# linwe2012/CourseComputationalPhotography

Hardware: AMD Instinct MI355X
Metric: Gauss-Seidel pixel-updates/s on WxH 5-point Poisson grid (higher is better)
Workload: dtype f64

## Files before the change

### coursecomputationalphotography_amd/csrc/ccp_grid.hip

```cpp
#include "ccp_grid_kernels.hpp"
#include "ccp_grid_fused.hpp"
#include "ccp_grid_fused_wide.hpp"
#include "ccp_grid_lex.hpp"
#include "ccp_cg.hpp"
#include "ccp_grid_cg.hpp"
#include "ccp_grid_mg_view.hpp"
#include "ccp_grid_blend.hpp"
#include "ccp_grid_weighted.hpp"
#include "ccp_comm.hpp"

#include <algorithm>
#include <functional>
#include <cstring>
#include <chrono>
#include <vector>

using namespace ccp;

constexpr int kEdgeRing = 64;

struct ccp_grid {
    ccp_grid_desc desc{};
    Geom geom{};
    int ghost_top = 0, ghost_bottom = 0;
    bool shrink_top = false, shrink_bottom = false;
    int device = 0;
    hipStream_t stream = nullptr;
    hipStream_t stream2 = nullptr;
    hipEvent_t ev_main = nullptr, ev_side = nullptr;
    unsigned long long *edge_counter = nullptr;
    unsigned long long *edge_flag = nullptr;
    unsigned long long edge_epoch = 0;
    unsigned *edge_timeout = nullptr;
    unsigned long long edge_timeout_ticks = 200000000ull;
    int wait_mode = 0;
    bool edge_signal = true;
    ccp_comm *comm = nullptr;
    std::vector<int> part;
    int up_rank = -1, down_rank = -1;
    int send_up = 0, send_down = 0;
    hipStream_t stream_comm = nullptr;
    hipEvent_t ev_comm = nullptr, ev_ready = nullptr;
    bool overlap = true;
    long exchanges = 0;
    DevBuf<double> x, b;
    DevBuf<double> cg_r, cg_p, cg_p2, cg_ap;
    DevBuf<CgState> cg_state;
    DevBuf<double> x_alt;
    bool allow_swap = false;
    bool masked = false;
    DevBuf<unsigned char> maskp, tile_live;
    DevBuf<int> tile_rows;
    DevBuf<unsigned char> mask_edge;
    bool mask_edge_known = false;
    int mask_border = -1;
    int live_T = -1, live_R = -1, live_lo = -1, live_hi = -1;
    long unknowns = 0;
    bool fuse = true;
    int multi = 0;
    DevBuf<unsigned> multi_words;
    bool xcd_swizzle = false;
    const char *trace_file = nullptr;
    DevBuf<unsigned long long> trace;
    bool short_edges = true;
    int side_rows_override = 0;
    int fuse_tmax = kFusedMaxT;
    int rows_per_chunk = 128;
    float tune_ms[kFusedMaxT + 1] = {0};
    int tune_rows[kFusedMaxT + 1] = {0};
    bool tuned = false;
    bool all_border = false;
    bool force_border = false;
    bool red_store_all = false;
    bool wide = true;
    DevBuf<double> partial;
    long partial_region = 0;
    DevBuf<double> small;
    DevBuf<unsigned> io_bad;
    DevBuf<double> sweep_sums;
    DevBuf<SolveState> state;
    DevBuf<int> redo_mask;
    DevBuf<double> lex_x, lex_b, lex_snap, lex_partial, lex_eps;
    DevBuf<unsigned> lex_progress, lex_ticket;
    DevBuf<double> lex_edges;
    int lex_mode = 3;
    int lex_tmax = 8;
    unsigned *lex_order_pin = nullptr;
    unsigned *lex_order_dev = nullptr;
    size_t lex_order_pin_cap = 0;
    size_t lex_order_count = 0;
    int lex_order_groups = 0, lex_order_strips = 0, lex_order_depth = 0;
    LexGeom lexg{};
    DevBuf<double> stage;
    long stage_rows = 0;
    int half_sweeps_since_refresh = 0;
    hipEvent_t ev0 = nullptr, ev1 = nullptr;
    hipEvent_t ev_r0 = nullptr, ev_r1 = nullptr;
    long region_launches = 0;
    long region_iterations = 0;
    float last_ms = 0.f;
    int last_launches = 0;
    bool timing_pending = false;
    int cpt = 2;
    int rows_per_block = 32;
    MgHierarchy *mg = nullptr;
    bool weighted = false;
    bool has_op = false;
    DevBuf<double> wop, wpart;
    int mg_kind = CCP_MG_HIERARCHY_GALERKIN;
};

namespace {

constexpr int kWeightedApplyBlocks = 1024;

int edge_timeout_status(const ccp_grid *g)
{
    if (g->edge_timeout && __atomic_load_n(g->edge_timeout, __ATOMIC_ACQUIRE) != 0) {
        if (getenv("CCP_GS_DEBUG")) fprintf(stderr, "[ccp_gs] an edge hand-off timed out: ghost rows may hold rows that were not final\n");
        return CCP_ERR_STATE;
    }
    return CCP_OK;
}

int bind(ccp_grid *g)
{
    if (!g) return CCP_ERR_BAD_ARG;
    if (hipSetDevice(g->device) != hipSuccess) return CCP_ERR_NO_DEVICE;
    return edge_timeout_status(g);
}

int not_weighted(const ccp_grid *g)
{
    if (!g) return CCP_ERR_BAD_ARG;
    return g->weighted ? CCP_ERR_UNSUPPORTED : CCP_OK;
}

long sweep_blocks_x(const ccp_grid *g) { return (g->geom.pitch + (long)kBlock * g->cpt - 1) / ((long)kBlock * g->cpt); }

void choose_tiling(ccp_grid *g)
{
    const long bx = sweep_blocks_x(g);
    long r = (long)g->geom.local_rows * bx * g->desc.channels / 4096;
    r = std::max<long>(4, std::min<long>(64, r));
    g->rows_per_block = (int)r;
}

template <bool L1>
int launch_half_sweep(ccp_grid *g, int c, int l_lo, int l_hi, const int *active)
{
    if (l_hi <= l_lo) return CCP_OK;
    const Geom &geo = g->geom;
    const int rpb = g->rows_per_block;
    dim3 grid((unsigned)sweep_blocks_x(g), (unsigned)((l_hi - l_lo + rpb - 1) / rpb), (unsigned)g->desc.channels);
    dim3 block(kBlock);
    double *part = g->partial.p + (long)c * g->partial_region;
#define CCP_LAUNCH_SWEEP(CPT_, SHFL_)                                                                          \
// ... 140 lines not shown
    }
    CCP_TRY(masked_tile_census(g, P, T));
    static const bool clip_rows = !(getenv("CCP_GS_MASK_ROWS") && atoi(getenv("CCP_GS_MASK_ROWS")) == 0);
    const int *rows_p = clip_rows ? g->tile_rows.p : nullptr;
    if (l1 == 2 && T > kMaskedMaxCheckedT) return CCP_ERR_BAD_ARG;
    constexpr int TMC = T <= kMaskedMaxCheckedT ? T : 1;
    if (l1 == 2) hipLaunchKernelGGL((k_fused_sweep_masked<TMC, 2, kFusedUnroll>), grid, dim3(kBlock), 0, g->stream, P, g->tile_live.p, rows_p);
    else if (l1 == 1) hipLaunchKernelGGL((k_fused_sweep_masked<TM, 1, kFusedUnroll>), grid, dim3(kBlock), 0, g->stream, P, g->tile_live.p, rows_p);
    else if (!store_red) hipLaunchKernelGGL((k_fused_sweep_masked<TM, 0, kFusedUnroll, false>), grid, dim3(kBlock), 0, g->stream, P, g->tile_live.p, rows_p);
    else hipLaunchKernelGGL((k_fused_sweep_masked<TM, 0, kFusedUnroll>), grid, dim3(kBlock), 0, g->stream, P, g->tile_live.p, rows_p);
    CCP_HIP(hipGetLastError());
    g->last_launches++;
    g->region_launches++;
    g->region_iterations += T;
    return CCP_OK;
}

template <int T>
int launch_fused_t(ccp_grid *g, const double *xin, double *xout, int st_lo, int st_hi, const int *active,
                   int l1 = 0, long *l1_blocks = nullptr, int rows_override = 0, int edge_rows = 0, bool *signalled = nullptr,
                   bool store_red = true)
{
    FusedParams P;
    P.xin = xin;
    P.xout = xout;
    P.b = g->b.p;
    P.g = g->geom;
    P.st_lo = st_lo;
    P.st_hi = st_hi;
    P.rows_per_chunk = rows_override > 0 ? rows_override : ((g->tuned && g->tune_rows[T] > 0) ? g->tune_rows[T] : g->rows_per_chunk);
    const int U = fused_useful_px(T);
    P.n_strips = (g->geom.W + U - 1) / U;
    P.partial = g->partial.p;
    P.partial_border = g->partial.p + g->partial_region;
    P.active = active;
    P.xcd_swizzle = g->xcd_swizzle ? 1 : 0;
    const bool want_edge = edge_rows > 0 && l1 == 0 && active == nullptr && g->edge_counter && g->edge_signal;
    P.mask = g->maskp.p;
    if (l1 != 0 || edge_rows > 0) store_red = true;
    if (g->masked) return launch_fused_masked<T>(g, P, l1, l1_blocks, store_red);
    fused_tile_counts(g, T, P, want_edge ? edge_rows : 0);
    const int waves = kBlock / kWave;
    const int edge_chunks = std::min(P.nb_top + P.nb_bot, P.n_chunks);
    const int edge_strips = std::min(P.ns_left + P.ns_right, P.n_strips);
    {
        const int HS = 2 * T, R = P.rows_per_chunk;
        int sr = std::max(16, (R + 2 * HS) * 2 / 5 - 2 * HS);
        sr += sr & 1;
        if (g->side_rows_override > 0) sr = std::max(2, g->side_rows_override);
        P.side_rows = std::min(sr, R);
        P.side_subs = (R + P.side_rows - 1) / P.side_rows;
        P.side_rows_edge = std::min(P.side_rows, 16);
        if (P.first_edge || P.last_edge)
            P.side_subs = std::max(P.side_subs, (std::max(P.first_rows, P.last_rows) + P.side_rows_edge - 1) / P.side_rows_edge);
    }
    const long n_border = (long)edge_chunks * (P.n_strips - edge_strips) + (long)P.n_chunks * edge_strips * P.side_subs;
    const bool any_plain = edge_chunks < P.n_chunks && edge_strips < P.n_strips;
    dim3 grid((unsigned)((P.n_strips + waves - 1) / waves), (unsigned)P.n_chunks, (unsigned)g->desc.channels);
    dim3 bgrid((unsigned)((n_border + waves - 1) / waves), 1, (unsigned)g->desc.channels);
    if (l1_blocks) {
        l1_blocks[0] = any_plain ? (long)grid.x * grid.y : 0;
        l1_blocks[1] = n_border ? (long)bgrid.x : 0;
    }
    if (l1 == 2 && T > kFusedMaxCheckedT) return CCP_ERR_BAD_ARG;
    const bool edge = want_edge && (P.first_edge || P.last_edge);
    P.edge_counter = g->edge_counter;
    P.edge_flag = g->edge_flag;
    P.edge_epoch = g->edge_epoch;
    P.edge_target = 0;
    if (edge) {
        long waves_expected = 0;
        for (int c = 0; c < P.n_chunks; c += std::max(1, P.n_chunks - 1)) {
            if (!fused_is_edge_chunk(P, c)) continue;
            int ra, rb;
            fused_chunk_rows(P, c, ra, rb);
            const int subs = std::min(P.side_subs, (rb - ra + P.side_rows_edge - 1) / P.side_rows_edge);
            waves_expected += (P.n_strips - edge_strips) + (long)edge_strips * subs;
        }
        P.edge_target = (unsigned long long)waves_expected * g->desc.channels;
        if (g->edge_epoch % kEdgeRing == 0) CCP_HIP(hipMemsetAsync(g->edge_counter, 0, sizeof(unsigned long long) * kEdgeRing, g->stream));
        P.edge_counter = g->edge_counter + (g->edge_epoch % kEdgeRing);
    }
    if (signalled) *signalled = edge;
    const bool wide = T == kWideT && g->wide && l1 == 0 && !edge && any_plain;
    const int wx0 = P.ns_left * U, wx1 = (P.n_strips - P.ns_right) * U;
    const int n_wide = wide ? (wx1 - wx0 + wide_useful_px(T) - 1) / wide_useful_px(T) : 0;
    const dim3 wgrid((unsigned)((n_wide + kWideWaves - 1) / kWideWaves), (unsigned)(P.n_chunks - edge_chunks), (unsigned)g->desc.channels);
    const dim3 pgrid = wide ? wgrid : grid;
    const size_t trace_plain = (size_t)pgrid.x * pgrid.y * pgrid.z * waves * 4, trace_border = (size_t)bgrid.x * bgrid.z * waves * 4;
    unsigned long long *trace_p = nullptr, *trace_b = nullptr;
    if (g->trace_file) {
        if (g->trace.n < trace_plain + trace_border) CCP_TRY(g->trace.alloc(trace_plain + trace_border));
        CCP_HIP(hipMemsetAsync(g->trace.p, 0, (trace_plain + trace_border) * sizeof(unsigned long long), g->stream));
        trace_p = g->trace.p;
        trace_b = g->trace.p + trace_plain;
    }
    P.trace = trace_b;
    constexpr int TC = T <= kFusedMaxCheckedT ? T : 1;
    hipStream_t bstream = g->stream2;
    if (n_border) {
        CCP_HIP(hipEventRecord(g->ev_main, g->stream));
        CCP_HIP(hipStreamWaitEvent(bstream, g->ev_main, 0));
    }
    if (n_border && edge) {
        hipLaunchKernelGGL((k_fused_border<T, 0, kFusedUnroll, true>), bgrid, dim3(kBlock), 0, bstream, P, g->force_border ? 1 : 0);
    }
    if (any_plain) {
        P.trace = trace_p;
        if (l1 == 2) hipLaunchKernelGGL((k_fused_sweep<TC, 2, kFusedUnroll>), grid, dim3(kBlock), 0, g->stream, P);
        else if (l1 == 1) hipLaunchKernelGGL((k_fused_sweep<T, 1, kFusedUnroll>), grid, dim3(kBlock), 0, g->stream, P);
        else if (edge) hipLaunchKernelGGL((k_fused_sweep<T, 0, kFusedUnroll, true>), grid, dim3(kBlock), 0, g->stream, P);
        else if (wide && !store_red) hipLaunchKernelGGL((k_fused_sweep_wide<kWideT, false>), wgrid, dim3(kBlock), 0, g->stream, P, wx0, wx1, n_wide);
        else if (wide) hipLaunchKernelGGL((k_fused_sweep_wide<kWideT, true>), wgrid, dim3(kBlock), 0, g->stream, P, wx0, wx1, n_wide);
        else if (!store_red) hipLaunchKernelGGL((k_fused_sweep<T, 0, kFusedUnroll, false, false>), grid, dim3(kBlock), 0, g->stream, P);
        else hipLaunchKernelGGL((k_fused_sweep<T, 0, kFusedUnroll>), grid, dim3(kBlock), 0, g->stream, P);
    }
    if (n_border) {
        const int fb = g->force_border ? 1 : 0;
        P.trace = trace_b;
        if (l1 == 2) hipLaunchKernelGGL((k_fused_border<TC, 2, kFusedUnroll>), bgrid, dim3(kBlock), 0, bstream, P, fb);
        else if (l1 == 1) hipLaunchKernelGGL((k_fused_border<T, 1, kFusedUnroll>), bgrid, dim3(kBlock), 0, bstream, P, fb);
        else if (!edge) hipLaunchKernelGGL((k_fused_border<T, 0, kFusedUnroll>), bgrid, dim3(kBlock), 0, bstream, P, fb);
        CCP_HIP(hipEventRecord(g->ev_side, bstream));
        CCP_HIP(hipStreamWaitEvent(g->stream, g->ev_side, 0));
    }
    CCP_HIP(hipGetLastError());
    if (g->trace_file) {
        CCP_HIP(hipStreamSynchronize(g->stream));
        std::vector<unsigned long long> host(trace_plain + trace_border);
        CCP_HIP(hipMemcpy(host.data(), g->trace.p, host.size() * sizeof(unsigned long long), hipMemcpyDeviceToHost));
        if (FILE *f = fopen(g->trace_file, "ab")) {
            const unsigned long long head[8] = {0x43435054524143ull, (unsigned long long)T, pgrid.x, pgrid.y, pgrid.z, bgrid.x, (unsigned long long)host.size(),
                                                (unsigned long long)P.rows_per_chunk};
            fwrite(head, sizeof(head), 1, f);
            fwrite(host.data(), sizeof(unsigned long long), host.size(), f);
            fclose(f);
        }
    }
    g->last_launches++;
    g->region_launches++;
    g->region_iterations += T;
    return CCP_OK;
}

template <int T>
int launch_fused_multi_t(ccp_grid *g, int n_passes, const double *xin, double *xout, const int *st_lo, const int *st_hi, int red_skip = 0)
{
    if (n_passes < 2 || n_passes > kMultiMaxPasses || g->trace_file) return CCP_ERR_UNSUPPORTED;
    if (g->masked && T > kMaskedMaxT) return CCP_ERR_UNSUPPORTED;
    FusedMultiParams M{};
    FusedParams &P = M.P;
    P.xin = xin;
    P.xout = xout;
    P.b = g->b.p;
    P.g = g->geom;
    P.st_lo = st_lo[0];
    P.st_hi = st_hi[0];
    P.rows_per_chunk = (g->tuned && g->tune_rows[T] > 0) ? g->tune_rows[T] : g->rows_per_chunk;
    const int U = fused_useful_px(T);
    P.n_strips = (g->geom.W + U - 1) / U;
    P.partial = g->partial.p;
    P.partial_border = g->partial.p + g->partial_region;
    P.active = nullptr;
    P.xcd_swizzle = 0;
    P.mask = g->maskp.p;
    P.trace = nullptr;
    const int HS = 2 * T;
    if (g->masked) {
        P.first_rows = P.last_rows = P.first_edge = P.last_edge = 0;
        P.n_chunks = (P.st_hi - P.st_lo + P.rows_per_chunk - 1) / P.rows_per_chunk;
// ... 268 lines not shown
    g->timing_pending = true;
    return CCP_OK;
}

template <bool TO_DEVICE>
int transfer_rows(ccp_grid *g, double *dev_base, int channel, double *rows, int first_row, int n_rows)
{
    CCP_TRY(bind(g));
    if (!rows || channel < 0 || channel >= g->desc.channels || n_rows < 0) return CCP_ERR_BAD_ARG;
    const int img_lo = g->geom.y0, img_hi = g->geom.y0 + g->geom.local_rows;
    if (first_row < img_lo || first_row + n_rows > img_hi) return CCP_ERR_BAD_ARG;
    const int W = g->desc.width;
    int done = 0;
    while (done < n_rows) {
        const int chunk = (int)std::min<long>(g->stage_rows, n_rows - done);
        const int l_first = first_row + done - g->geom.y0;
        dim3 grid((unsigned)((W + kBlock - 1) / kBlock), (unsigned)chunk);
        const size_t bytes = (size_t)chunk * W * sizeof(double);
        double *host = rows + (size_t)done * W;
        if (TO_DEVICE) {
            CCP_HIP(hipMemcpyAsync(g->stage.p, host, bytes, hipMemcpyHostToDevice, g->stream));
            hipLaunchKernelGGL((k_convert<true>), grid, dim3(kBlock), 0, g->stream, dev_base, g->stage.p,
                               g->geom, channel, l_first, W);
            CCP_HIP(hipGetLastError());
        } else {
            hipLaunchKernelGGL((k_convert<false>), grid, dim3(kBlock), 0, g->stream, dev_base, g->stage.p,
                               g->geom, channel, l_first, W);
            CCP_HIP(hipGetLastError());
            CCP_HIP(hipMemcpyAsync(host, g->stage.p, bytes, hipMemcpyDeviceToHost, g->stream));
        }
        CCP_HIP(hipStreamSynchronize(g->stream));
        done += chunk;
    }
    return edge_timeout_status(g);
}

}

extern "C" {

int ccp_grid_create(const ccp_grid_desc *d, ccp_grid **out)
try {
    if (!d || !out) return CCP_ERR_BAD_ARG;
    *out = nullptr;
    if (d->width < 1 || d->height < 1 || d->channels < 1 || d->channels > kMaxChannels) return CCP_ERR_BAD_ARG;
    if (d->row_begin < 0 || d->row_count < 1 || d->row_begin + d->row_count > d->height || d->ghost < 0)
        return CCP_ERR_BAD_ARG;
    if ((long)d->width * d->height > 0x7fffffffL) return CCP_ERR_BAD_ARG;
    if ((d->flags & CCP_GRID_WEIGHTED) &&
        ((d->flags & CCP_GRID_DIRICHLET_MASK) || d->ghost != 0 || d->row_begin != 0 || d->row_count != d->height))
        return CCP_ERR_UNSUPPORTED;
    CCP_TRY(select_device(d->device));
    ccp_grid *g = new (std::nothrow) ccp_grid();
    if (!g) return CCP_ERR_ALLOC;
    g->desc = *d;
    g->device = d->device;
    g->ghost_top = d->row_begin > 0 ? std::min(d->ghost, d->row_begin) : 0;
    g->ghost_bottom = (d->row_begin + d->row_count < d->height) ? std::min(d->ghost, d->height - d->row_begin - d->row_count) : 0;
    Geom &geo = g->geom;
    geo.W = d->width;
    geo.H = d->height;
    geo.y0 = d->row_begin - g->ghost_top;
    g->shrink_top = geo.y0 > 0;
    g->shrink_bottom = d->row_begin + d->row_count + g->ghost_bottom < d->height;
    geo.local_rows = g->ghost_top + d->row_count + g->ghost_bottom;
    geo.own_lo = g->ghost_top;
    geo.own_hi = g->ghost_top + d->row_count;
    geo.pitch = (((long)d->width + 1) / 2 + 15) / 16 * 16;
    geo.ch_stride = (long)geo.local_rows * 2 * geo.pitch;
    g->cpt = 2;
    if (const char *e = getenv("CCP_GS_FUSE")) g->fuse = atoi(e) != 0;
    if (const char *e = getenv("CCP_GS_SHORT_EDGES")) g->short_edges = atoi(e) != 0;
    if (const char *e = getenv("CCP_GS_XCD")) g->xcd_swizzle = atoi(e) != 0;
    if (const char *e = getenv("CCP_GS_MULTI")) g->multi = atoi(e);
    if (const char *e = getenv("CCP_GS_TRACE_FILE")) g->trace_file = e[0] ? e : nullptr;
    if (const char *e = getenv("CCP_GS_SIDE_ROWS")) g->side_rows_override = atoi(e);
    if (const char *e = getenv("CCP_GS_LEX_MODE"))
        g->lex_mode = strcmp(e, "planes") == 0 ? 0 : 3;
    if (const char *e = getenv("CCP_GS_TMAX")) g->fuse_tmax = std::max(1, std::min(kFusedMaxT, atoi(e)));
    if (const char *e = getenv("CCP_GS_ALL_BORDER")) g->all_border = atoi(e) != 0;
    if (const char *e = getenv("CCP_GS_FORCE_BORDER")) g->force_border = atoi(e) != 0;
    if (const char *e = getenv("CCP_GS_RED_STORE")) g->red_store_all = atoi(e) != 0;
    if (const char *e = getenv("CCP_GS_WIDE")) g->wide = atoi(e) != 0;
    if (const char *e = getenv("CCP_GS_CHUNK")) g->rows_per_chunk = std::max(1, atoi(e));
    choose_tiling(g);
    g->masked = (d->flags & CCP_GRID_DIRICHLET_MASK) != 0;
    if (g->masked) {
        g->fuse_tmax = std::min(g->fuse_tmax, kMaskedMaxT);
        if (!getenv("CCP_GS_CHUNK")) g->rows_per_chunk = 160;
    }

    const size_t elems = (size_t)geo.ch_stride * d->channels;
    int st = g->x.alloc(elems);
    if (st == CCP_OK && g->masked) {
        st = g->maskp.alloc((size_t)geo.ch_stride);
        if (st == CCP_OK && hipMemset(g->maskp.p, 0, (size_t)geo.ch_stride) != hipSuccess) st = CCP_ERR_HIP;
        if (st == CCP_OK) st = g->mask_edge.alloc(2 * (size_t)d->width);
        if (st == CCP_OK && hipMemset(g->mask_edge.p, 0, 2 * (size_t)d->width) != hipSuccess) st = CCP_ERR_HIP;
    }
    if (st == CCP_OK) st = g->b.alloc(elems);
    g->weighted = (d->flags & CCP_GRID_WEIGHTED) != 0;
    if (st == CCP_OK && g->weighted) {
        st = g->wop.alloc(4 * (size_t)geo.ch_stride);
        if (st == CCP_OK && hipMemset(g->wop.p, 0, 4 * sizeof(double) * (size_t)geo.ch_stride) != hipSuccess) st = CCP_ERR_HIP;
        if (st == CCP_OK) st = g->wpart.alloc(4 * (size_t)d->channels * kWeightedApplyBlocks);
    }
    const size_t part = (size_t)((geo.pitch + 2L * kBlock - 1) / (2L * kBlock)) * geo.local_rows * d->channels * 2 * 2 + 64;
    g->partial_region = (long)(part / 2);
    if (st == CCP_OK) st = g->partial.alloc(part);
    if (st == CCP_OK) st = g->small.alloc(4 * kMaxChannels);
    if (st == CCP_OK) st = g->io_bad.alloc(1);
    if (st == CCP_OK) st = g->state.alloc(1);
    g->stage_rows = std::max<long>(1, std::min<long>(geo.local_rows, (8L << 20) / d->width));
    if (st == CCP_OK) st = g->stage.alloc((size_t)g->stage_rows * d->width);
    if (st == CCP_OK && (hipEventCreate(&g->ev0) != hipSuccess || hipEventCreate(&g->ev1) != hipSuccess)) st = CCP_ERR_HIP;
    if (st == CCP_OK && (hipStreamCreateWithFlags(&g->stream2, hipStreamNonBlocking) != hipSuccess ||
                         hipEventCreateWithFlags(&g->ev_main, hipEventDisableTiming) != hipSuccess ||
                         hipEventCreateWithFlags(&g->ev_side, hipEventDisableTiming) != hipSuccess))
        st = CCP_ERR_HIP;
    if (st == CCP_OK && (g->ghost_top || g->ghost_bottom)) {
        int can_wait = 0;
        (void)hipDeviceGetAttribute(&can_wait, hipDeviceAttributeCanUseStreamWaitValue, g->device);
        g->wait_mode = can_wait ? 0 : 1;
        if (const char *e = getenv("CCP_GS_EDGE_WAIT")) g->wait_mode = (strcmp(e, "spin") == 0) ? 1 : (can_wait ? 0 : 1);
        if (const char *e = getenv("CCP_GS_EDGE_SIGNAL")) g->edge_signal = atoi(e) != 0;
        if (hipMalloc(reinterpret_cast<void **>(&g->edge_counter), sizeof(unsigned long long) * kEdgeRing) != hipSuccess ||
            hipExtMallocWithFlags(reinterpret_cast<void **>(&g->edge_flag), sizeof(unsigned long long), hipMallocSignalMemory) != hipSuccess ||
            hipMemset(g->edge_counter, 0, sizeof(unsigned long long) * kEdgeRing) != hipSuccess ||
            hipMemset(g->edge_flag, 0, sizeof(unsigned long long)) != hipSuccess)
            st = CCP_ERR_HIP;
        if (const char *e = getenv("CCP_GS_EDGE_TIMEOUT_TICKS")) g->edge_timeout_ticks = strtoull(e, nullptr, 10);
    }
    if (st == CCP_OK && hipHostMalloc(reinterpret_cast<void **>(&g->edge_timeout), sizeof(unsigned), hipHostMallocMapped) != hipSuccess) st = CCP_ERR_HIP;
    if (g->edge_timeout) *g->edge_timeout = 0;
    if (st == CCP_OK && (hipMemset(g->x.p, 0, elems * sizeof(double)) != hipSuccess ||
                         hipMemset(g->b.p, 0, elems * sizeof(double)) != hipSuccess))
        st = CCP_ERR_HIP;
    if (st != CCP_OK) {
        ccp_grid_destroy(g);
        return st;
    }
    *out = g;
    return CCP_OK;
} CCP_ABI_CATCH

int ccp_grid_destroy(ccp_grid *g)
try {
    if (!g) return CCP_OK;
    (void)hipSetDevice(g->device);
    if (g->ev0) (void)hipEventDestroy(g->ev0);
    if (g->ev1) (void)hipEventDestroy(g->ev1);
    if (g->ev_r0) (void)hipEventDestroy(g->ev_r0);
    if (g->ev_r1) (void)hipEventDestroy(g->ev_r1);
    if (g->ev_main) (void)hipEventDestroy(g->ev_main);
    if (g->ev_side) (void)hipEventDestroy(g->ev_side);
    if (g->stream2) {
        (void)hipStreamSynchronize(g->stream2);
        (void)hipStreamDestroy(g->stream2);
    }
    if (g->stream_comm) {
        (void)hipStreamSynchronize(g->stream_comm);
        (void)hipStreamDestroy(g->stream_comm);
    }
    if (g->ev_comm) (void)hipEventDestroy(g->ev_comm);
    if (g->ev_ready) (void)hipEventDestroy(g->ev_ready);
    if (g->edge_counter) (void)hipFree(g->edge_counter);
// ... 2208 lines not shown
```

### coursecomputationalphotography_amd/csrc/ccp_grid_fused.hpp

```cpp
#pragma once

#include "ccp_grid_kernels.hpp"

namespace ccp {

#ifndef CCP_FUSED_MAX_T
#define CCP_FUSED_MAX_T 8
#endif
constexpr int kFusedMaxT = CCP_FUSED_MAX_T;
constexpr int kFusedMaxCheckedT = 8;
#ifndef CCP_FUSED_UNROLL
#define CCP_FUSED_UNROLL 2
#endif
constexpr int kFusedUnroll = CCP_FUSED_UNROLL;
#ifndef CCP_FUSED_LAND
#define CCP_FUSED_LAND 2
#endif
constexpr int kFusedLand = CCP_FUSED_LAND;
constexpr int kStripLanes = kWave;

__host__ __device__ constexpr int fused_halo_px(int T) { return 2 * T; }
__host__ __device__ constexpr int fused_useful_px(int T) { return 2 * kStripLanes - 4 * T; }

__device__ __forceinline__ double lane_prev(double v)
{
    int lo = __double2loint(v), hi = __double2hiint(v);
    lo = __builtin_amdgcn_update_dpp(0, lo, 0x138, 0xf, 0xf, true);
    hi = __builtin_amdgcn_update_dpp(0, hi, 0x138, 0xf, 0xf, true);
    return __hiloint2double(hi, lo);
}
__device__ __forceinline__ double lane_next(double v)
{
    int lo = __double2loint(v), hi = __double2hiint(v);
    lo = __builtin_amdgcn_update_dpp(0, lo, 0x130, 0xf, 0xf, true);
    hi = __builtin_amdgcn_update_dpp(0, hi, 0x130, 0xf, 0xf, true);
    return __hiloint2double(hi, lo);
}

struct FusedParams {
    const double *__restrict__ xin;
    double *__restrict__ xout;
    const double *__restrict__ b;
    Geom g;
    int st_lo, st_hi;
    int rows_per_chunk;
    int first_rows, last_rows;
    int n_strips;
    double *__restrict__ partial;
    const int *__restrict__ active;
    int n_chunks;
    int nb_top, nb_bot, ns_left, ns_right;
    int side_rows, side_subs;
    int side_rows_edge;
    double *__restrict__ partial_border;
    const unsigned char *__restrict__ mask;
    int first_edge, last_edge;
    int xcd_swizzle;
    unsigned long long *__restrict__ trace;
    unsigned long long *__restrict__ edge_counter;
    unsigned long long *__restrict__ edge_flag;
    unsigned long long edge_target, edge_epoch;
};

__host__ __device__ __forceinline__ int fused_chunk_of(const FusedParams &P, int y)
{
    const int n_e = P.first_edge + P.last_edge;
    if (y < n_e) return (P.first_edge && y == 0) ? 0 : P.n_chunks - 1;
    return y - n_e + P.first_edge;
}

__host__ __device__ __forceinline__ bool fused_is_edge_chunk(const FusedParams &P, int chunk)
{
    return (P.first_edge && chunk == 0) || (P.last_edge && chunk == P.n_chunks - 1);
}

__device__ __forceinline__ void fused_signal_edge(const FusedParams &P)
{
    __builtin_amdgcn_fence(__ATOMIC_RELEASE, "agent");
    if ((threadIdx.x & (kWave - 1)) == 0) {
        const unsigned long long old = __hip_atomic_fetch_add(P.edge_counter, 1ull, __ATOMIC_RELAXED, __HIP_MEMORY_SCOPE_AGENT);
        if (old + 1 == P.edge_target)
            __hip_atomic_store(P.edge_flag, P.edge_epoch, __ATOMIC_RELEASE, __HIP_MEMORY_SCOPE_SYSTEM);
    }
}

__device__ __forceinline__ void fused_tile_coords(const FusedParams &P, unsigned &bx, unsigned &by, unsigned &bz)
{
    bx = blockIdx.x;
    by = blockIdx.y;
    bz = blockIdx.z;
    if (P.xcd_swizzle) {
        const unsigned gx = gridDim.x, gy = gridDim.y;
        const unsigned n = gx * gy * gridDim.z;
        const unsigned id = bx + gx * (by + gy * bz);
        const unsigned xcd = id & 7u, k = id >> 3;
        const unsigned q = n >> 3, r = n & 7u;
        const unsigned tile = xcd * q + (xcd < r ? xcd : r) + k;
        bx = tile % gx;
        const unsigned t = tile / gx;
        by = t % gy;
        bz = t / gy;
    }
}

__device__ __forceinline__ void fused_trace_begin(const FusedParams &P, unsigned long long &t0)
{
    if (P.trace) t0 = wall_clock64();
}
__device__ __forceinline__ void fused_trace_end(const FusedParams &P, unsigned long long t0, long slot, int chunk, int sx, int ch, int kernel)
{
    if (P.trace && (threadIdx.x & (kWave - 1)) == 0) {
        unsigned long long *r = P.trace + 4 * slot;
        r[0] = t0;
        r[1] = wall_clock64();
        r[2] = (unsigned long long)__builtin_amdgcn_s_getreg((4 << 0) | (0 << 6) | (31 << 11))
               | ((unsigned long long)__builtin_amdgcn_s_getreg((20 << 0) | (0 << 6) | (3 << 11)) << 32);
        r[3] = (unsigned long long)(unsigned)chunk | ((unsigned long long)(unsigned)sx << 16) | ((unsigned long long)ch << 32) |
               ((unsigned long long)kernel << 40);
    }
}

__host__ __device__ __forceinline__ void fused_chunk_rows(const FusedParams &P, int c, int &ra, int &rb)
{
    if (P.first_rows > 0 && c == 0) {
        ra = P.st_lo;
        rb = P.st_lo + P.first_rows;
    } else if (P.last_rows > 0 && c == P.n_chunks - 1) {
        ra = P.st_hi - P.last_rows;
        rb = P.st_hi;
    } else {
        const int k = c - (P.first_rows > 0 ? 1 : 0);
        const int end = P.st_hi - P.last_rows;
        ra = P.st_lo + P.first_rows + k * P.rows_per_chunk;
        rb = ra + P.rows_per_chunk < end ? ra + P.rows_per_chunk : end;
    }
}

template <int T, int UNR>
struct FusedWindow {
    static_assert(UNR > 0 && UNR % 2 == 0, "row parity must be a compile-time constant per unrolled step");
// ... 633 lines not shown
```

### coursecomputationalphotography_amd/csrc/ccp_grid_fused_wide.hpp

```cpp
#pragma once

#include "ccp_grid_fused.hpp"

namespace ccp {

constexpr int kWideT = 8;
constexpr int kWideRing = 20;
constexpr int kWideWaves = kBlock / kWave;
__host__ __device__ constexpr int wide_useful_px(int T) { return 4 * kStripLanes - 4 * T; }

typedef unsigned int u32x4 __attribute__((ext_vector_type(4)));
typedef double d2 __attribute__((ext_vector_type(2)));

__device__ __forceinline__ d2 buf_load2(__amdgpu_buffer_rsrc_t rs, unsigned voff)
{
    return __builtin_bit_cast(d2, __builtin_amdgcn_raw_buffer_load_b128(rs, (int)voff, 0, 0));
}
__device__ __forceinline__ void buf_store2(d2 v, __amdgpu_buffer_rsrc_t rs, unsigned voff)
{
    __builtin_amdgcn_raw_buffer_store_b128(__builtin_bit_cast(u32x4, v), rs, (int)voff, 0, 0);
}

struct WideCtx {
    const double *__restrict__ xin;
    double *__restrict__ xout;
    const double *__restrict__ bb;
    unsigned ld_r, ld_k;
    unsigned st_r, st_k;
    int ra, rb;
    int m0, m1;
    d2 *ring;
};

__device__ __forceinline__ void wide_load_row(const WideCtx &cx, const Geom &g, int q, d2 (&dst)[4])
{
    const bool exists = q >= cx.m0 && q < cx.m1;
    const __amdgpu_buffer_rsrc_t rx = row_rsrc(cx.xin, g, q, exists), rbb = row_rsrc(cx.bb, g, q, exists);
    dst[0] = buf_load2(rx, cx.ld_r);
    dst[1] = buf_load2(rx, cx.ld_k);
    dst[2] = buf_load2(rbb, cx.ld_r);
    dst[3] = buf_load2(rbb, cx.ld_k);
}

__host__ __device__ constexpr int wide_slot(int k) { return ((k % kWideRing) + kWideRing) % kWideRing; }

template <int T, bool STORE_RED, int NT, int PH>
__device__ __forceinline__ void wide_step(d2 (&wr)[NT], d2 (&wk)[NT], const WideCtx &cx, const Geom &g, int f, int i)
{
    using Win = FusedWindow<T, 2>;
    constexpr int HS = Win::HS;
#pragma unroll
    for (int h = 1; h <= HS; ++h) {
        const int sr = Win::slot(i, h), su = Win::slot(i, h + 1), sd = Win::slot(i, h - 1);
        const int c = (h - 1) & 1;
        const int p = ((i - h + 2 * HS + 2) + c) & 1;
        const d2 up = c ? wr[su] : wk[su];
        const d2 dn = c ? wr[sd] : wk[sd];
        const d2 o = c ? wr[sr] : wk[sr];
        double la, ra, lb, rb;
        if (p == 0) {
            la = lane_prev(o.y); ra = o.x; lb = o.x; rb = o.y;
        } else {
            la = o.x; ra = o.y; lb = o.y; rb = lane_next(o.x);
        }
        const d2 bq = cx.ring[wide_slot(PH + i - h) * 2 * kWave + c * kWave];
        d2 nv;
        nv.x = __builtin_fma(((up.x + la) + ra) + dn.x, 0.25, bq.x);
        nv.y = __builtin_fma(((up.y + lb) + rb) + dn.y, 0.25, bq.y);
        if (c) wk[sr] = nv; else wr[sr] = nv;
    }
    {
        const int r = f - HS;
        const int sr = Win::slot(i, HS);
        const __amdgpu_buffer_rsrc_t ro = row_rsrc(cx.xout, g, r, r >= cx.ra && r < cx.rb);
        if constexpr (STORE_RED) buf_store2(wr[sr], ro, cx.st_r);
        buf_store2(wk[sr], ro, cx.st_k);
    }
    __builtin_amdgcn_sched_barrier(0);
}

template <int NT>
__device__ __forceinline__ void wide_place(d2 (&wr)[NT], d2 (&wk)[NT], const WideCtx &cx, int s0, int slot, const d2 (&row)[4])
{
    wr[s0] = row[0];
    wk[s0] = row[1];
    cx.ring[slot * 2 * kWave] = row[2] * 0.25;
    cx.ring[slot * 2 * kWave + kWave] = row[3] * 0.25;
}

template <int T, bool STORE_RED, int NT, int PH>
// ... 5 lines not shown
#pragma unroll
    for (int i = 0; i < G; ++i) wide_load_row(cx, g, fb + 2 * G + i, landing[i]);
    __builtin_amdgcn_sched_barrier(0);
#pragma unroll
    for (int i = 0; i < G; ++i) {
        if (i == 0) wide_step<T, STORE_RED, NT, PH>(wr, wk, cx, g, fb, 0);
        else wide_step<T, STORE_RED, NT, PH>(wr, wk, cx, g, fb + 1, 1);
    }
#pragma unroll
    for (int s = 0; s + G < NT; ++s) {
        wr[s] = wr[s + G];
        wk[s] = wk[s + G];
    }
#pragma unroll
    for (int i = 0; i < G; ++i) wide_place(wr, wk, cx, Win::slot(i, 0), wide_slot(PH + G + i), arrived[i]);
}

template <int T, bool STORE_RED, int NT, int PH>
__device__ __forceinline__ void wide_turn(d2 (&wr)[NT], d2 (&wk)[NT], const WideCtx &cx, const Geom &g, int fb,
                                          d2 (&la)[2][4], d2 (&lb)[2][4])
{
    if constexpr (PH < kWideRing) {
        if constexpr ((PH / 2) % 2 == 0) wide_trip<T, STORE_RED, NT, PH>(wr, wk, cx, g, fb, la, lb);
        else wide_trip<T, STORE_RED, NT, PH>(wr, wk, cx, g, fb, lb, la);
        wide_turn<T, STORE_RED, NT, PH + 2>(wr, wk, cx, g, fb + 2, la, lb);
    }
}

template <int T, bool STORE_RED>
__device__ __forceinline__ void fused_wave_wide(const double *__restrict__ xin, double *__restrict__ xout,
                                                const double *__restrict__ bb, const Geom &g, int wx0, int wx1, int sw,
                                                int ra, int rb, d2 *ring)
{
    static_assert(T % 2 == 0, "the lane pairs line up with the stored columns only for an even depth");
    constexpr int G = 2;
    static_assert(kWideRing % (2 * G) == 0 && kWideRing >= 2 * T + 2 * G, "the ring holds the rows a trip reads and the rows it lands");
    using Win = FusedWindow<T, G>;
    constexpr int HS = Win::HS, NT = Win::NT;
    const int lane = (int)(threadIdx.x & (kWave - 1));
    WideCtx cx;
    cx.xin = xin; cx.xout = xout; cx.bb = bb;
    cx.ring = ring + lane;
    const int x0 = wx0 + sw * wide_useful_px(T);
    const int x1 = min(x0 + wide_useful_px(T), wx1);
    const int ja = (x0 - fused_halo_px(T)) / 2 + 2 * lane;
    const bool col_ok = ja >= 0 && ja < g.pitch;
    const bool col_store = col_ok && 2 * ja >= x0 && 2 * ja + 3 < x1;
    cx.ld_r = col_ok ? (unsigned)ja * 8u : kLaneOut;
    cx.ld_k = col_ok ? (unsigned)(g.pitch + ja) * 8u : kLaneOut;
    cx.st_r = (STORE_RED && col_store) ? cx.ld_r : kLaneOut;
    cx.st_k = col_store ? cx.ld_k : kLaneOut;
    cx.ra = ra; cx.rb = rb;
    cx.m0 = max(ra - HS, 0);
    cx.m1 = min(rb + HS, g.local_rows);
    const int base = cx.m0 - ((g.y0 + cx.m0) & 1);
    const int f_end = rb - 1 + HS;

    d2 wr[NT], wk[NT];
    d2 la[G][4], lb[G][4];
#pragma unroll
    for (int s = 0; s < NT; ++s) wr[s] = wk[s] = d2{0.0, 0.0};
#pragma unroll
    for (int s = 0; s < kWideRing; ++s) {
        cx.ring[s * 2 * kWave] = d2{0.0, 0.0};
        cx.ring[s * 2 * kWave + kWave] = d2{0.0, 0.0};
    }
#pragma unroll
    for (int i = 0; i < G; ++i) wide_load_row(cx, g, base + i, la[i]);
#pragma unroll
    for (int i = 0; i < G; ++i) wide_load_row(cx, g, base + G + i, lb[i]);
#pragma unroll
    for (int i = 0; i < G; ++i) wide_place(wr, wk, cx, Win::slot(i, 0), i, la[i]);
    for (int fb = base; fb <= f_end; fb += kWideRing) wide_turn<T, STORE_RED, NT, 0>(wr, wk, cx, g, fb, la, lb);
}

template <int T, bool STORE_RED>
__global__ void __launch_bounds__(kBlock, 2)
k_fused_sweep_wide(FusedParams P, int wx0, int wx1, int n_wide)
{
    __shared__ d2 ring[kWideWaves][kWideRing * 2 * kWave];
    const int wave = __builtin_amdgcn_readfirstlane(threadIdx.x / kWave);
    unsigned bx, by, bz;
    fused_tile_coords(P, bx, by, bz);
    const int sw = (int)bx * kWideWaves + wave;
    const int ch = (int)bz;
    const int chunk = P.nb_top + (int)by;
    int ra, rb;
    fused_chunk_rows(P, chunk, ra, rb);
    const bool run = (P.active == nullptr) || (P.active[ch] != 0);
    if (run && sw < n_wide && ra < rb) {
        const Geom &g = P.g;
        const long off = (long)ch * g.ch_stride;
        unsigned long long t0 = 0;
        fused_trace_begin(P, t0);
        fused_wave_wide<T, STORE_RED>(P.xin + off, P.xout + off, P.b + off, g, wx0, wx1, sw, ra, rb, ring[wave]);
        fused_trace_end(P, t0, (((long)blockIdx.z * gridDim.y + blockIdx.y) * gridDim.x + blockIdx.x) * kWideWaves + wave, chunk, sw, ch, 3);
    }
}

}
```

Before: 2116 billion.

## Plan wide-sweep row segments with a cost model instead of fixed chunks

Result: faster. 2160 billion (median of 6 runs) (+2.1%).

```diff
diff --git a/coursecomputationalphotography_amd/csrc/ccp_grid.hip b/coursecomputationalphotography_amd/csrc/ccp_grid.hip
--- a/coursecomputationalphotography_amd/csrc/ccp_grid.hip
+++ b/coursecomputationalphotography_amd/csrc/ccp_grid.hip
@@ -73,6 +73,8 @@
     bool force_border = false;
     bool red_store_all = false;
     bool wide = true;
+    int cus = 0;
+    int wide_segments = -1;
     DevBuf<double> partial;
     long partial_region = 0;
     DevBuf<double> small;
@@ -379,10 +381,40 @@
         P.edge_counter = g->edge_counter + (g->edge_epoch % kEdgeRing);
     }
     if (signalled) *signalled = edge;
-    const bool wide = T == kWideT && g->wide && l1 == 0 && !edge && any_plain;
     const int wx0 = P.ns_left * U, wx1 = (P.n_strips - P.ns_right) * U;
-    const int n_wide = wide ? (wx1 - wx0 + wide_useful_px(T) - 1) / wide_useful_px(T) : 0;
-    const dim3 wgrid((unsigned)((n_wide + kWideWaves - 1) / kWideWaves), (unsigned)(P.n_chunks - edge_chunks), (unsigned)g->desc.channels);
+    const int n_wide = (T == kWideT && any_plain) ? (wx1 - wx0 + wide_useful_px(T) - 1) / wide_useful_px(T) : 0;
+    const bool wide = T == kWideT && g->wide && l1 == 0 && !edge && any_plain && n_wide > 0;
+    P.wide_y0 = P.wide_y1 = P.wide_nseg = P.wide_tiles = 0;
+    P.wide_stride = 1;
+    P.wide_h = 2;
+    if (wide) {
+        int t;
+        fused_chunk_rows(P, P.nb_top, P.wide_y0, t);
+        fused_chunk_rows(P, P.n_chunks - P.nb_bot - 1, t, P.wide_y1);
+        const int rows = P.wide_y1 - P.wide_y0;
+        const long per_seg = (long)n_wide * g->desc.channels;
+        WideBorder border;
+        for (int e = 0; e < edge_chunks; ++e) {
+            int ra, rb;
+            fused_chunk_rows(P, e < P.nb_top ? e : P.n_chunks - edge_chunks + e, ra, rb);
+            border.steps += (long)(rb - ra + 4 * T) * (P.n_strips - edge_strips);
+            border.longest = std::max(border.longest, rb - ra + 4 * T);
+        }
+        if (edge_strips > 0) {
+            border.steps += (long)P.n_chunks * edge_strips * P.side_subs * (P.side_rows + 4 * T);
+            border.longest = std::max(border.longest, P.side_rows + 4 * T);
+        }
+        border.steps *= g->desc.channels;
+        const int slots = kWideWaves * g->cus;
+        const WidePlan plan = g->wide_segments == 0 ? wide_plan_height(rows, P.rows_per_chunk)
+                              : g->wide_segments > 0 ? wide_plan_count(rows, g->wide_segments)
+                                                     : wide_plan(P.wide_y0, P.wide_y1, per_seg, slots, T, border);
+        P.wide_h = plan.h;
+        P.wide_nseg = plan.n_seg;
+        P.wide_stride = g->wide_segments == 0 ? (n_wide + kWideWaves - 1) / kWideWaves * kWideWaves : n_wide;
+        P.wide_tiles = P.wide_stride * plan.n_seg * g->desc.channels;
+    }
+    const dim3 wgrid((unsigned)((P.wide_tiles + kWideWaves - 1) / kWideWaves), 1, 1);
     const dim3 pgrid = wide ? wgrid : grid;
     const size_t trace_plain = (size_t)pgrid.x * pgrid.y * pgrid.z * waves * 4, trace_border = (size_t)bgrid.x * bgrid.z * waves * 4;
     unsigned long long *trace_p = nullptr, *trace_b = nullptr;
@@ -817,6 +849,11 @@
     if (const char *e = getenv("CCP_GS_FORCE_BORDER")) g->force_border = atoi(e) != 0;
     if (const char *e = getenv("CCP_GS_RED_STORE")) g->red_store_all = atoi(e) != 0;
     if (const char *e = getenv("CCP_GS_WIDE")) g->wide = atoi(e) != 0;
+    if (const char *e = getenv("CCP_GS_WIDE_SEGMENTS")) g->wide_segments = std::max(0, atoi(e));
+    if (hipDeviceGetAttribute(&g->cus, hipDeviceAttributeMultiprocessorCount, g->device) != hipSuccess || g->cus < 1) {
+        delete g;
+        return CCP_ERR_HIP;
+    }
     if (const char *e = getenv("CCP_GS_CHUNK")) g->rows_per_chunk = std::max(1, atoi(e));
     choose_tiling(g);
     g->masked = (d->flags & CCP_GRID_DIRICHLET_MASK) != 0;
diff --git a/coursecomputationalphotography_amd/csrc/ccp_grid_fused.hpp b/coursecomputationalphotography_amd/csrc/ccp_grid_fused.hpp
--- a/coursecomputationalphotography_amd/csrc/ccp_grid_fused.hpp
+++ b/coursecomputationalphotography_amd/csrc/ccp_grid_fused.hpp
@@ -56,6 +56,7 @@
     const unsigned char *__restrict__ mask;
     int first_edge, last_edge;
     int xcd_swizzle;
+    int wide_y0, wide_y1, wide_h, wide_nseg, wide_stride, wide_tiles;
     unsigned long long *__restrict__ trace;
     unsigned long long *__restrict__ edge_counter;
     unsigned long long *__restrict__ edge_flag;
diff --git a/coursecomputationalphotography_amd/csrc/ccp_grid_fused_wide.hpp b/coursecomputationalphotography_amd/csrc/ccp_grid_fused_wide.hpp
--- a/coursecomputationalphotography_amd/csrc/ccp_grid_fused_wide.hpp
+++ b/coursecomputationalphotography_amd/csrc/ccp_grid_fused_wide.hpp
@@ -1,11 +1,11 @@
 #pragma once
 
 #include "ccp_grid_fused.hpp"
+#include "ccp_wide_plan.hpp"
 
 namespace ccp {
 
 constexpr int kWideT = 8;
-constexpr int kWideRing = 20;
 constexpr int kWideWaves = kBlock / kWave;
 __host__ __device__ constexpr int wide_useful_px(int T) { return 4 * kStripLanes - 4 * T; }
 
@@ -177,20 +177,24 @@
     const int wave = __builtin_amdgcn_readfirstlane(threadIdx.x / kWave);
     unsigned bx, by, bz;
     fused_tile_coords(P, bx, by, bz);
-    const int sw = (int)bx * kWideWaves + wave;
-    const int ch = (int)bz;
-    const int chunk = P.nb_top + (int)by;
+    const int tile = (int)bx * kWideWaves + wave;
+    if (tile >= P.wide_tiles) return;
+    const int row = tile / P.wide_stride;
+    const int sw = tile - row * P.wide_stride;
+    if (sw >= n_wide) return;
+    const int ch = row / P.wide_nseg;
+    const int seg = row - ch * P.wide_nseg;
     int ra, rb;
-    fused_chunk_rows(P, chunk, ra, rb);
+    wide_segment_rows(P.wide_y0, P.wide_y1, P.wide_h, seg, ra, rb);
     const bool run = (P.active == nullptr) || (P.active[ch] != 0);
-    if (run && sw < n_wide && ra < rb) {
+    if (run && ra < rb) {
         const Geom &g = P.g;
         const long off = (long)ch * g.ch_stride;
         unsigned long long t0 = 0;
         fused_trace_begin(P, t0);
         fused_wave_wide<T, STORE_RED>(P.xin + off, P.xout + off, P.b + off, g, wx0, wx1, sw, ra, rb, ring[wave]);
-        fused_trace_end(P, t0, (((long)blockIdx.z * gridDim.y + blockIdx.y) * gridDim.x + blockIdx.x) * kWideWaves + wave, chunk, sw, ch, 3);
-    }
-}
-
-}
+        fused_trace_end(P, t0, tile, seg, sw, ch, 3);
+    }
+}
+
+}
diff --git a/coursecomputationalphotography_amd/csrc/ccp_wide_plan.hpp b/coursecomputationalphotography_amd/csrc/ccp_wide_plan.hpp
--- /dev/null
+++ b/coursecomputationalphotography_amd/csrc/ccp_wide_plan.hpp
@@ -0,0 +1,77 @@
+#pragma once
+
+#if defined(__HIPCC__)
+#define CCP_WIDE_PLAN_FN __host__ __device__ inline
+#else
+#define CCP_WIDE_PLAN_FN inline
+#endif
+
+namespace ccp {
+
+constexpr int kWideRing = 20;
+constexpr int kWideMinSegRows = 64;
+
+struct WidePlan {
+    int n_seg;
+    int h;
+};
+
+inline int wide_march_steps(int h, int T) { return (h + 4 * T + kWideRing - 1) / kWideRing * kWideRing; }
+
+struct WideBorder {
+    long steps = 0;
+    int longest = 0;
+};
+constexpr int kWideBorderPerCu = 2;
+constexpr int kWideBorderSlowNum = 5, kWideBorderSlowDen = 2;
+
+inline long wide_plan_cost(long tiles_per_segment, int n_seg, int h, int slots, int T, const WideBorder &border = WideBorder())
+{
+    const long tiles = tiles_per_segment * n_seg;
+    const long rounds = (tiles + slots - 1) / slots;
+    const long march = wide_march_steps(h, T);
+    const long free_cus = slots / 4 - (tiles + 3) / 4;
+    const bool hidden = border.steps == 0 || (rounds == 1 && kWideBorderPerCu * free_cus * march >= border.steps);
+    return rounds * march + (hidden ? 0 : (long)border.longest * kWideBorderSlowNum / kWideBorderSlowDen);
+}
+
+inline WidePlan wide_plan_height(int rows, int h)
+{
+    if (h < 1) h = 1;
+    return WidePlan{rows > 0 ? (rows + h - 1) / h : 0, h};
+}
+
+inline WidePlan wide_plan_count(int rows, int n)
+{
+    if (rows <= 0) return WidePlan{0, 2};
+    if (n < 1) n = 1;
+    int h = (rows + n - 1) / n;
+    h += h & 1;
+    return wide_plan_height(rows, h);
+}
+
+inline WidePlan wide_plan(int y0, int y1, long tiles_per_segment, int slots, int T, const WideBorder &border = WideBorder())
+{
+    const int rows = y1 - y0;
+    WidePlan best = wide_plan_count(rows, 1);
+    if (rows <= 0 || tiles_per_segment <= 0 || slots <= 0) return best;
+    long best_cost = wide_plan_cost(tiles_per_segment, best.n_seg, best.h, slots, T, border);
+    for (int n = 2; n <= rows / kWideMinSegRows; ++n) {
+        const WidePlan p = wide_plan_count(rows, n);
+        if (p.n_seg != n || p.h < kWideMinSegRows) continue;
+        const long cost = wide_plan_cost(tiles_per_segment, p.n_seg, p.h, slots, T, border);
+        if (cost < best_cost) {
+            best = p;
+            best_cost = cost;
+        }
+    }
+    return best;
+}
+
+CCP_WIDE_PLAN_FN void wide_segment_rows(int y0, int y1, int h, int s, int &ra, int &rb)
+{
+    ra = y0 + s * h;
+    rb = ra + h < y1 ? ra + h : y1;
+}
+
+}
```
